# DRL-Navigation/DDRL4NAV

Hardware: NVIDIA B200
Metric: PPO learner samples/s & batched policy actions/s at 1/2/4/8 B200 (higher is better)
Workload: dtype f32 (three tcgen05 kind::f16 products of scaled fp16 hi/lo splits, fp32 accumulate)

## Files before the change

### ddrl4nav_b200/_lib.py

```python
import ctypes as C
import os

_HERE = os.path.dirname(os.path.abspath(__file__))
LIB_PATH = os.environ.get("DDRL_LIB_PATH") or os.path.join(_HERE, "libddrl_b200.so")


class DDRLError(RuntimeError):
    pass


class NetDesc(C.Structure):
    _fields_ = [("arch", C.c_int32), ("in_ch", C.c_int32), ("act_dim", C.c_int32), ("dist", C.c_int32),
                ("shared", C.c_int32), ("feat", C.c_int32), ("gemm_mode", C.c_int32), ("laser_ch", C.c_int32)]


class PPOHparams(C.Structure):
    _fields_ = [("ppo_clip", C.c_float), ("dual_clip", C.c_float), ("v_coef", C.c_float), ("ent_coef", C.c_float),
                ("max_grad_norm", C.c_float), ("clip_grad", C.c_int32), ("smooth_l1", C.c_int32),
                ("lr", C.c_float), ("lr_actor", C.c_float), ("lr_critic", C.c_float),
                ("beta1", C.c_float), ("beta2", C.c_float), ("adam_eps", C.c_float)]


class GatherJob(C.Structure):
    _fields_ = [("src", C.c_void_p), ("dst", C.c_void_p), ("row_bytes", C.c_int64), ("src_stride", C.c_int64),
# ... 44 lines not shown
    "ddrl_net_num_params": (_L, [_P]),
    "ddrl_net_tensor_info": (_I, [_P, _I, C.c_char_p, _I, C.POINTER(_L), C.POINTER(_I), C.POINTER(_L)]),
    "ddrl_net_bind": (_I, [_P, _P, _P, _P, _P]),
    "ddrl_net_params_changed": (_I, [_P]),
    "ddrl_net_set_extra_critics": (_I, [_P, _I, C.POINTER(_P), C.POINTER(_P), C.POINTER(_P), C.POINTER(_P), C.POINTER(_I)]),
    "ddrl_net_num_obs": (_I, [_P]),
    "ddrl_net_obs_elems": (_L, [_P, _I]),
    "ddrl_net_forward": (_I, [_P, C.POINTER(_P), _I, _I, _P, _P, _P, _P, _P, _P]),
    "ddrl_net_encode": (_I, [_P, C.POINTER(_P), _I, _I, _I, _P, _P]),
    "ddrl_net_backward": (_I, [_P, C.POINTER(_P), _I, _I, _I, _P, _P, _P, _P, C.POINTER(PPOHparams), _I, _P]),
    "ddrl_net_backward_segment": (_I, [_P, C.POINTER(_P), _I, _I, _I, _P, _P, _P, _P, C.POINTER(PPOHparams), _I, _I, C.POINTER(_I), _P]),
    "ddrl_net_tensor_segment": (_I, [_P, _I]),
    "ddrl_net_backward_minibatch": (_I, [_P, C.POINTER(_P), _I, _I, _I, _P, _P, _P, _P, C.POINTER(PPOHparams), _P]),
    "ddrl_gather_rows": (_I, [_P, _I, C.POINTER(GatherJob), _I, _P]),
    "ddrl_set_deterministic": (_I, [_I]),
    "ddrl_peer_allreduce_flag_bytes": (_I, []),
    "ddrl_peer_allreduce_f32": (_I, [C.POINTER(_P), _P, C.POINTER(_P), _I, _I, C.c_int64, C.c_int64, C.c_uint32, _P]),
    "ddrl_net_clip_adam": (_I, [_P, _I, C.POINTER(PPOHparams), _P, _P]),
    "ddrl_net_workspace_bytes": (_L, [_P]),
}

_lib = None


def load():
    global _lib
    if _lib is not None:
        return _lib
    if not os.path.exists(LIB_PATH):
        raise DDRLError(
# ... 34 lines not shown
```

### ddrl4nav_b200/csrc/tc3.cu

```cuda
#include <cuda.h>
#include <cuda_fp16.h>

#include <algorithm>
#include <cstdlib>
#include <cstring>
#include <mutex>
#include <vector>

#include "common.cuh"
#include "layer_ops.h"
#include "prep_kernels.cuh"
#include "tc_ptx.cuh"

namespace ddrl {

constexpr int T3_BM = 128;
constexpr int T3_BK = 64;
constexpr int T3_CHUNK = 4;

__device__ unsigned long long g_tc3_wait[96];
#ifdef TC3_TIMING
#define T3_T0 const long long _t0 = clock64()
#define T3_ACC(acc) acc += clock64() - _t0
#define T3_WAIT(bar, par, acc) do { T3_T0; mbar_wait(bar, par); T3_ACC(acc); } while (0)
// ... 31 lines not shown
  int act, atomic, vec_store;
  int tma_store;
  int tma_mask;
  int presplit;
  int b_resident;
  int m_tiles, n_tiles;
  const float* amax_a;
  const float* amax_b;
  float* amax_out;
  unsigned int* bits_out;
  const unsigned int* bits_in;
  float* colsum;
  float* colsum2;
  int colsum_split;
  unsigned int* det_ctr;
  TcTap tap;
};

template <bool SCALED = true>
__device__ __forceinline__ void t3_split2(float x0, float x1, float s, uint32_t& hi, uint32_t& lo) {
  const float y0 = SCALED ? x0 * s : x0, y1 = SCALED ? x1 * s : x1;
  asm("cvt.rn.satfinite.f16x2.f32 %0, %1, %2;" : "=r"(hi) : "f"(y1), "f"(y0));
  const float2 f = __half22float2(*reinterpret_cast<const __half2*>(&hi));
  const float r0 = (y0 - f.x) * T3_LO, r1 = (y1 - f.y) * T3_LO;
  asm("cvt.rn.satfinite.f16x2.f32 %0, %1, %2;" : "=r"(lo) : "f"(r1), "f"(r0));
}

__device__ __forceinline__ void umma_f16_ts(uint32_t tmem_d, uint32_t tmem_a, uint64_t db, uint32_t idesc, uint32_t accumulate) {
  asm volatile(
      "{\n"
      ".reg .pred p;\n"
      "setp.ne.b32 p, %4, 0;\n"
      "tcgen05.mma.cta_group::1.kind::f16 [%0], [%1], %2, %3, p;\n"
      "}" ::"r"(tmem_d), "r"(tmem_a), "l"(db), "r"(idesc), "r"(accumulate) : "memory");
}

__device__ __forceinline__ void umma_f16_ss(uint32_t tmem_d, uint64_t da, uint64_t db, uint32_t idesc, uint32_t accumulate) {
  asm volatile(
      "{\n"
      ".reg .pred p;\n"
      "setp.ne.b32 p, %4, 0;\n"
      "tcgen05.mma.cta_group::1.kind::f16 [%0], %1, %2, %3, p;\n"
      "}" ::"r"(tmem_d), "l"(da), "l"(db), "r"(idesc), "r"(accumulate) : "memory");
}

template <int BN>
struct T3Cfg {
  static constexpr int A_SUB = T3_BM * 128;
  static constexpr int A_BYTES = 2 * A_SUB;
  static constexpr int B_BYTES = BN * 128;
  static constexpr int STAGE_BYTES = A_BYTES + 2 * B_BYTES;
  static constexpr int STAGES = BN <= 32 ? 5 : (BN <= 64 ? 4 : 3);
  static constexpr bool FOLD = BN <= 64;
  static constexpr int SA = BN <= 32 ? 4 : (BN <= 64 ? 3 : 2);
  static constexpr int NEPI = BN <= 32 ? 4 : 8;
  static constexpr int NSG = BN <= 64 ? 2 : 1;
  static constexpr int EPI0 = 4 + 4 * NSG;
  static constexpr int THREADS = (EPI0 + NEPI) * 32;
  static constexpr int COLS = BN / (NEPI / 4);
  static constexpr int TM_MAIN0 = 0, TM_MAIN1 = FOLD ? 2 * BN : BN, TM_CORR = FOLD ? 4 * BN : 2 * BN, TM_A = FOLD ? 5 * BN : 3 * BN;
  static constexpr int TMEM_COLS = 512;
  static constexpr int NBARS = 2 * STAGES + SA + 7;
  static constexpr int STG_OFF = STAGES * STAGE_BYTES;
  static constexpr int BAR_OFF = STG_OFF + NEPI * 4096;
  static constexpr int BIAS_OFF = BAR_OFF + 256;
  static constexpr int SMEM = 1024 + BIAS_OFF + BN * 4;
  static_assert(NBARS * 8 + 16 <= 256, "barrier block");
  static_assert(SMEM <= 232448, "shared memory budget");
  static_assert(TM_A + SA * 64 <= 512, "TMEM budget");
  static_assert(STAGES > SA, "the stage barrier of K block it - SA releases TMEM slot it % SA");
};

template <int BN>
__global__ void __launch_bounds__(T3Cfg<BN>::THREADS, 1)
tc3_kernel(const __grid_constant__ CUtensorMap tmA, const __grid_constant__ CUtensorMap tmBhi,
           const __grid_constant__ CUtensorMap tmBlo, const __grid_constant__ CUtensorMap tmA2,
           const __grid_constant__ CUtensorMap tmC, const __grid_constant__ CUtensorMap tmC2,
           const __grid_constant__ CUtensorMap tmM, const __grid_constant__ CUtensorMap tmM2, Tc3Args g) {
  using Cfg = T3Cfg<BN>;
  constexpr int S = Cfg::STAGES, SA = Cfg::SA;
  extern __shared__ uint8_t smem_dyn[];
  uint8_t* smem = smem_dyn + ((1024u - (smem_u32(smem_dyn) & 1023u)) & 1023u);
  uint64_t* bars = reinterpret_cast<uint64_t*>(smem + Cfg::BAR_OFF);
  uint64_t* bar_full = bars;
  uint64_t* bar_empty = bars + S;
  uint64_t* bar_aready = bars + 2 * S;
  uint64_t* bar_mfull = bars + 2 * S + SA;
  uint64_t* bar_mfree = bar_mfull + 2;
  uint64_t* bar_cfull = bar_mfull + 4;
  uint64_t* bar_cfree = bar_mfull + 5;
  uint64_t* bar_mask = bar_mfull + 6;
  uint32_t* tmem_slot = reinterpret_cast<uint32_t*>(bars + Cfg::NBARS);
  const int warp = threadIdx.x >> 5, lane = threadIdx.x & 31;
  const TcTap& tp = g.tap;
  const bool tapA = tp.mode != 0;

  if (warp == 0 && lane == 0) {
    mbar_init(smem_u32(bar_mask), 1);
    for (int s = 0; s < S; ++s) { mbar_init(smem_u32(bar_full + s), 1); mbar_init(smem_u32(bar_empty + s), 2); }
    for (int a = 0; a < SA; ++a) mbar_init(smem_u32(bar_aready + a), 4);
    for (int b = 0; b < 2; ++b) { mbar_init(smem_u32(bar_mfull + b), 1); mbar_init(smem_u32(bar_mfree + b), Cfg::NEPI); }
    mbar_init(smem_u32(bar_cfull), 1);
    mbar_init(smem_u32(bar_cfree), Cfg::NEPI);
    asm volatile("fence.mbarrier_init.release.cluster;" ::: "memory");
  }
  if (warp == 2) {
    asm volatile("tcgen05.alloc.cta_group::1.sync.aligned.shared::cta.b32 [%0], %1;" ::"r"(smem_u32(tmem_slot)),
                 "r"((uint32_t)Cfg::TMEM_COLS) : "memory");
    asm volatile("tcgen05.relinquish_alloc_permit.cta_group::1.sync.aligned;" ::: "memory");
  }
  tc_fence_before();
  __syncthreads();
  tc_fence_after();
  const uint32_t tmem_base = *tmem_slot;

  const int total_tiles = g.m_tiles * g.n_tiles;
  const int tile_step = (int)gridDim.x, tile_first = (int)blockIdx.x;
  const int nkb = g.kb_total;
  const bool ps = g.presplit != 0;
  const bool odd_tail = tapA && !ps && (tp.nslices & 1);

  if (warp == 0) {
    uint32_t it = 0;
    T3_ROLE_BEGIN
    for (int tile = tile_first; tile < total_tiles; tile += tile_step) {
      const int mt = tile / g.n_tiles, nt = tile - mt * g.n_tiles;
      const int m0 = mt * T3_BM, n0 = nt * BN;
      int b0 = 0, y0 = 0;
      const bool ph2 = tapA && mt >= tp.tiles1;
      if (tapA) {
        if (!ph2) { b0 = (mt / tp.tpi) * tp.nb; y0 = (mt % tp.tpi) * tp.ny * tp.sy - tp.py; }
        else { b0 = (mt - tp.tiles1) * tp.nb2; y0 = tp.y2 * tp.sy - tp.py; }
      }
      int cc = 0, kw = 0, kh = 0;
      for (int i = 0; i < nkb; ++i, ++it) {
        const uint32_t s = it % S;
        T3_WAITL(smem_u32(bar_empty + s), ((it / S) & 1) ^ 1, w0);
        const bool load_b = !g.b_resident || it < (uint32_t)S;
        const uint32_t b_tx = load_b ? 2u * Cfg::B_BYTES : 0u;
        if (elect_one()) {
          const uint32_t full = smem_u32(bar_full + s);
          const uint32_t a_dst = smem_u32(smem) + s * Cfg::STAGE_BYTES, bh_dst = a_dst + Cfg::A_BYTES, bl_dst = bh_dst + Cfg::B_BYTES;
          const int k = i * T3_BK;
          if (ps) {
            if (!tapA) {
              mbar_expect_tx(full, Cfg::A_BYTES + b_tx);
              tma_load_2d(&tmA, full, a_dst, k, m0);
// ... 28 lines not shown
        if (tapA) {
#pragma unroll
          for (int j = 0; j < 2; ++j) {
            if (ps && j == 1) break;
            if (++cc == tp.cpb) { cc = 0; if (++kw == tp.KW) { kw = 0; ++kh; } }
          }
        }
      }
    }
    T3_ROLE_END(0, true);
  } else if (warp == 1 || warp == 3) {
    const bool chunk_role = warp == 1;
    const uint32_t idesc = (1u << 4) | ((uint32_t)(BN >> 3) << 17) | ((uint32_t)(T3_BM >> 4) << 24);
    const uint32_t idesc2 = (1u << 4) | ((uint32_t)((2 * BN) >> 3) << 17) | ((uint32_t)(T3_BM >> 4) << 24);
    const uint32_t smem_base = smem_u32(smem);
    const uint32_t t_corr = tmem_base + Cfg::TM_CORR;
    uint32_t it = 0, ch = 0, tl = 0;
    T3_ROLE_BEGIN
    for (int tile = tile_first; tile < total_tiles; tile += tile_step, ++tl) {
      for (int i = 0; i < nkb; ++i, ++it) {
        const uint32_t s = it % S, a = it % SA;
        const uint32_t buf = ch & 1;
        const bool first_in_chunk = (i % T3_CHUNK) == 0;
        const bool last_in_chunk = (i % T3_CHUNK) == T3_CHUNK - 1 || i == nkb - 1;
        const int ksteps = (odd_tail && i == nkb - 1) ? 2 : 4;
        if (chunk_role) { if (first_in_chunk) T3_WAIT(smem_u32(bar_mfree + buf), ((ch >> 1) & 1) ^ 1, w0); }
        else if (i == 0) T3_WAIT(smem_u32(bar_cfree), (tl & 1) ^ 1, w0);
        if (ps) T3_WAIT(smem_u32(bar_full + s), (it / S) & 1, w1);
        else T3_WAIT(smem_u32(bar_aready + a), (it / SA) & 1, w1);
        tc_fence_after();
        T3_SECTION_BEGIN;
        if (elect_one()) {
          const uint32_t b_hi = smem_base + s * Cfg::STAGE_BYTES + Cfg::A_BYTES, b_lo = b_hi + Cfg::B_BYTES;
          const uint32_t a_hi = tmem_base + Cfg::TM_A + a * 64, a_lo = a_hi + 32;
          const uint64_t dbh0 = umma_desc(b_hi, 16, 1024, 2);
          if (ps) {
            const uint32_t sa_hi = smem_base + s * Cfg::STAGE_BYTES;
            const uint64_t dah0 = umma_desc(sa_hi, 16, 1024, 2), dal0 = umma_desc(sa_hi + Cfg::A_SUB, 16, 1024, 2);
            if (chunk_role) {
              const uint32_t t_main = tmem_base + (buf ? Cfg::TM_MAIN1 : Cfg::TM_MAIN0);
#pragma unroll
              for (int k4 = 0; k4 < 4; ++k4)
                umma_f16_ss(t_main, dah0 + k4 * 2, dbh0 + k4 * 2, Cfg::FOLD ? idesc2 : idesc, (!first_in_chunk || k4 != 0) ? 1u : 0u);
              umma_commit(smem_u32(bar_empty + s));
              if (last_in_chunk) umma_commit(smem_u32(bar_mfull + buf));
            } else {
              const uint64_t dbl0 = umma_desc(b_lo, 16, 1024, 2);
#pragma unroll
              for (int k4 = 0; k4 < 4; ++k4) {
                umma_f16_ss(t_corr, dal0 + k4 * 2, dbh0 + k4 * 2, idesc, (i | k4) != 0 ? 1u : 0u);
                if (!Cfg::FOLD) umma_f16_ss(t_corr, dah0 + k4 * 2, dbl0 + k4 * 2, idesc, 1u);
              }
              umma_commit(smem_u32(bar_empty + s));
              if (i == nkb - 1) umma_commit(smem_u32(bar_cfull));
            }
          } else if (chunk_role) {
            const uint32_t t_main = tmem_base + (buf ? Cfg::TM_MAIN1 : Cfg::TM_MAIN0);
#pragma unroll
            for (int k4 = 0; k4 < 4; ++k4) {
              if (k4 >= ksteps) break;
              umma_f16_ts(t_main, a_hi + k4 * 8, dbh0 + k4 * 2, Cfg::FOLD ? idesc2 : idesc, (!first_in_chunk || k4 != 0) ? 1u : 0u);
            }
            umma_commit(smem_u32(bar_empty + s));
            if (last_in_chunk) umma_commit(smem_u32(bar_mfull + buf));
          } else {
            const uint64_t dbl0 = umma_desc(b_lo, 16, 1024, 2);
#pragma unroll
            for (int k4 = 0; k4 < 4; ++k4) {
              if (k4 >= ksteps) break;
              umma_f16_ts(t_corr, a_lo + k4 * 8, dbh0 + k4 * 2, idesc, (i | k4) != 0 ? 1u : 0u);
              if (!Cfg::FOLD) umma_f16_ts(t_corr, a_hi + k4 * 8, dbl0 + k4 * 2, idesc, 1u);
            }
            umma_commit(smem_u32(bar_empty + s));
            if (i == nkb - 1) umma_commit(smem_u32(bar_cfull));
          }
        }
        __syncwarp();
        T3_SECTION_END(w2);
        if (last_in_chunk) ++ch;
      }
    }
    T3_ROLE_END(chunk_role ? 1 : 2, true);
  } else if (warp >= 4 && warp < Cfg::EPI0) {
    const int q = (warp - 4) & 3, grp = (warp - 4) >> 2;
    const uint32_t t_lane = (uint32_t)(q * 32) << 16;
    float sA, sA_inv;
    t3_scale(__ldg(g.amax_a), sA, sA_inv);
    const bool unit_scale = sA == 1.f;
    const int row = q * 32 + lane;
    uint32_t it = 0;
    T3_ROLE_BEGIN
    for (int tile = ps ? total_tiles : tile_first; tile < total_tiles; tile += tile_step) {
      for (int i = 0; i < nkb; ++i, ++it) {
        const int s = it % S, a = it % SA;
// ... 119 lines not shown
  } else if (warp >= Cfg::EPI0) {
    const int e = warp - Cfg::EPI0;
    const int q = e & 3, half = e >> 2;
    const uint32_t t_lane = (uint32_t)(q * 32) << 16;
    const uint32_t col0 = half * Cfg::COLS;
    float sA, sA_inv, sB, sB_inv;
    t3_scale(__ldg(g.amax_a), sA, sA_inv);
    t3_scale(__ldg(g.amax_b), sB, sB_inv);
    float run_max = 0.f;
    uint32_t ch = 0, tl = 0, mround = 0;
    float s_pre = 1.f, s_out = sA_inv * sB_inv;
    if (!(s_out >= 1e-30f && s_out <= 1e30f)) { s_pre = sA_inv; s_out = sB_inv; }
    const int r = q * 32 + lane;
    int ryb1 = 0, ryb2 = 0;
    const bool need_off = !g.tma_store || g.bits_out != nullptr || g.bits_in != nullptr;
    const int rx = (tapA && need_off) ? r % tp.Xn : 0;
    if (tapA) {
      const int t1 = r / tp.Xn;
      ryb1 = (t1 % tp.ny) | ((t1 / tp.ny) << 16);
      if (tp.ny2 > 0) ryb2 = (t1 % tp.ny2) | ((t1 / tp.ny2) << 16);
    }
    float* bias_s = reinterpret_cast<float*>(smem + Cfg::BIAS_OFF);
    const int et = e * 32 + lane;
    T3_ROLE_BEGIN
    for (int tile = tile_first; tile < total_tiles; tile += tile_step, ++tl) {
      const int mt = tile / g.n_tiles, nt = tile - mt * g.n_tiles;
      const int m0 = mt * T3_BM, n0 = nt * BN;
      int cy = 0, cb = 0;
      if (tapA) {
        const bool ph2 = mt >= tp.tiles1;
        cb = ph2 ? (mt - tp.tiles1) * tp.nb2 : (mt / tp.tpi) * tp.nb;
        cy = ph2 ? tp.y2 : (mt % tp.tpi) * tp.ny;
      }
      const bool masked = g.tma_store && g.tma_mask;
      float bias_r = 0.f;
      if (g.tma_store && et < BN && g.bias != nullptr && n0 + et < g.N) bias_r = __ldg(g.bias + n0 + et);
      const bool ph2e = tapA && mt >= tp.tiles1;
      const int ryb = ph2e ? ryb2 : ryb1;
      const bool rvalid = tapA ? (r < (ph2e ? tp.rows2 : tp.rows) && cb + (ryb >> 16) < tp.Bn && cy + (ryb & 0xffff) < tp.Yn)
                               : (m0 + r) < g.M;
      const bool fused = tapA && tp.ncls > 1;
      long long roff = 0;
      int py = 0, px = 0;
      if (need_off) {
        if (tapA) {
          const int yy = ryb & 0xffff, bb = ryb >> 16;
          roff = (long long)(cb + bb) * tp.osb + (long long)(cy + yy) * tp.osy + (long long)rx * tp.osx;
          if (fused) { px = rx * tp.out_s; py = (cy + yy) * tp.out_s; }
        } else {
          roff = (long long)(m0 + r) * g.sCm;
        }
      }
      uint32_t mw[Cfg::COLS / 32];
#pragma unroll
      for (int p = 0; p < Cfg::COLS / 32; ++p) mw[p] = 0u;
// ... 31 lines not shown
            continue;
          }
          tmem_ld32(tmem_base + t_lane + (buf ? Cfg::TM_MAIN1 : Cfg::TM_MAIN0) + col0 + j0, v);
#pragma unroll
          for (int j = 0; j < 32; ++j) acc[j0 + j] += v[j];
          if (Cfg::FOLD) {
            tmem_ld32(tmem_base + t_lane + (buf ? Cfg::TM_MAIN1 : Cfg::TM_MAIN0) + BN + col0 + j0, v);
#pragma unroll
            for (int j = 0; j < 32; ++j) acc[j0 + j] = fmaf(v[j], T3_LO_INV, acc[j0 + j]);
          }
        }
        tc_fence_before();
        __syncwarp();
        if (lane == 0) mbar_arrive(smem_u32(bar_mfree + buf));
      }
      T3_WAITL(smem_u32(bar_cfull), tl & 1, w1);
      tc_fence_after();
#pragma unroll
      for (int j0 = 0; j0 < Cfg::COLS; j0 += 32) {
        float v[32];
        tmem_ld32(tmem_base + t_lane + Cfg::TM_CORR + col0 + j0, v);
#pragma unroll
        for (int j = 0; j < 32; ++j) acc[j0 + j] = fmaf(v[j], T3_LO_INV, acc[j0 + j]);
      }
      tc_fence_before();
      __syncwarp();
      if (lane == 0) mbar_arrive(smem_u32(bar_cfree));
      if (s_pre != 1.f) {
#pragma unroll
        for (int j = 0; j < Cfg::COLS; ++j) acc[j] *= s_pre;
      }
      T3_SECTION_BEGIN;
      const float neg_slope = g.act == 3 ? 0.f : 0.01f;
      if (!g.tma_store) {
#pragma unroll
        for (int j = 0; j < Cfg::COLS; ++j) acc[j] *= s_out;
      }
      if (g.tma_store) {
        float* stg = reinterpret_cast<float*>(smem + Cfg::STG_OFF) + e * 1024;
        const bool relu = g.act == 1;
        const float slope = g.act == 2 ? 0.01f : 1.f;
        const bool has_bias = g.bias != nullptr;
// ... 219 lines not shown
#pragma unroll
      for (int o = 16; o > 0; o >>= 1) run_max = fmaxf(run_max, __shfl_xor_sync(0xffffffffu, run_max, o));
      if (lane == 0 && run_max > 0.f) atomicMax(reinterpret_cast<unsigned int*>(g.amax_out), __float_as_uint(run_max));
    }
  }
  tc_fence_before();
  __syncthreads();
  if (warp == 2) {
    asm volatile("tcgen05.dealloc.cta_group::1.sync.aligned.b32 %0, %1;" ::"r"(tmem_base), "r"((uint32_t)Cfg::TMEM_COLS)
                 : "memory");
  }
}

struct Tc3Maps { CUtensorMap a, bhi, blo, a2, c, c2, m, m2; };

template <int BN>
static int launch3(const Tc3Maps& m, const Tc3Args& g, dim3 grid, cudaStream_t s) {
  using Cfg = T3Cfg<BN>;
  static bool attr_done_dev[64] = {};
  bool& attr_done = attr_done_dev[current_device_index()];
  if (!attr_done) {
    DDRL_CUDA(cudaFuncSetAttribute(tc3_kernel<BN>, cudaFuncAttributeMaxDynamicSharedMemorySize, Cfg::SMEM));
    attr_done = true;
  }
  static const bool no_bres = [] { const char* e = getenv("DDRL_TC3_NO_BRES"); return e && e[0] == '1'; }();
  Tc3Args ga = g;
  ga.b_resident = (!no_bres && g.n_tiles == 1 && g.kb_total >= 1 && Cfg::STAGES % g.kb_total == 0) ? 1 : 0;
  tc3_kernel<BN><<<grid, Cfg::THREADS, Cfg::SMEM, s>>>(m.a, m.bhi, m.blo, m.a2, m.c, m.c2, m.m, m.m2, ga);
  prof_work(2.0 * g.M * (double)g.N * g.K * (g.tap.work_scale > 0.f ? g.tap.work_scale : 1.f));
  if (g_prof_on && g_prof_shapes) {
    char nm[96];
    snprintf(nm, sizeof(nm), "%s3[fwd,M=%d,N=%d,K=%d,g=%d]", g.tap.mode ? "conv_tc" : "gemm_tc", g.M, g.N, g.K,
             (int)(grid.x * grid.y * grid.z));
    DDRL_LAUNCHED(prof_intern(nm));
    return DDRL_OK;
  }
  DDRL_LAUNCHED("tc3_kernel");
  return DDRL_OK;
}

static int launch3_bn(int bn, const Tc3Maps& m, const Tc3Args& g, dim3 grid, cudaStream_t s) {
  switch (bn) {
    case 128: return launch3<128>(m, g, grid, s);
    case 64: return launch3<64>(m, g, grid, s);
    default: return launch3<32>(m, g, grid, s);
  }
}
static const bool g_t3_tma_store = [] { const char* e = getenv("DDRL_TC3_TMA_STORE"); return !(e && e[0] == '0'); }();
static const bool g_t3_tma_dgrad = [] { const char* e = getenv("DDRL_TC3_TMA_DGRAD"); return !(e && e[0] == '0'); }();

static inline int pick_bn3(int N) { return N > 64 ? 128 : (N > 32 ? 64 : 32); }
static inline bool al16(const void* p) { return (reinterpret_cast<uintptr_t>(p) & 15) == 0; }
// ... 3 lines not shown
  const unsigned long long strides[1] = {(unsigned long long)ldb16 * 2};
  const unsigned box[2] = {64u, (unsigned)bn}, estr[2] = {1u, 1u};
  return tc_encode_tiled(m, true, 2, base, dims, strides, box, estr, true);
}

static int make_map_nhwc16(CUtensorMap* m, const void* plane, const ConvOp& o, int nx, int ny, int nb) {
  const unsigned long long dims[4] = {(unsigned long long)o.Ctot, (unsigned long long)o.Win, (unsigned long long)o.Hin, (unsigned long long)o.Bn};
  const unsigned long long strides[3] = {(unsigned long long)o.Ctot * 2, (unsigned long long)o.Win * o.Ctot * 2,
                                         (unsigned long long)o.Hin * o.Win * o.Ctot * 2};
  const unsigned box[4] = {64u, (unsigned)((nx - 1) * o.sx + 1), (unsigned)((ny - 1) * o.sy + 1), (unsigned)nb};
  const unsigned estr[4] = {1u, (unsigned)o.sx, (unsigned)o.sy, 1u};
  return tc_encode_tiled(m, true, 4, plane, dims, strides, box, estr, true);
}
static inline bool presplit_ok(const ConvOp& o, const void* hi, const void* lo) {
  return hi && lo && al16(hi) && al16(lo) && o.Cin % 64 == 0 && o.Ctot % 8 == 0 && o.c_off % 8 == 0;
}

__global__ void __launch_bounds__(256) presplit_kernel(const float* __restrict__ x, long long n8, const float* __restrict__ amax,
                                                       uint4* __restrict__ hi, uint4* __restrict__ lo) {
  float sA, sA_inv;
  t3_scale(__ldg(amax), sA, sA_inv);
  const float4* x4 = reinterpret_cast<const float4*>(x);
  for (long long i = (long long)blockIdx.x * blockDim.x + threadIdx.x; i < n8; i += (long long)gridDim.x * blockDim.x) {
    const float4 a = __ldg(x4 + 2 * i), b = __ldg(x4 + 2 * i + 1);
    uint4 h, l;
    t3_split2(a.x, a.y, sA, h.x, l.x); t3_split2(a.z, a.w, sA, h.y, l.y);
    t3_split2(b.x, b.y, sA, h.z, l.z); t3_split2(b.z, b.w, sA, h.w, l.w);
    hi[i] = h; lo[i] = l;
  }
}
// ... 100 lines not shown
  const int bn = pick_bn3(N);
  Tc3Args g;
  memset(&g, 0, sizeof(g));
  tc_tap_common(g.tap, o, T3_BM, true);
  g.tap.osb = osb; g.tap.osy = osy; g.tap.osx = osx;
  if (cls && cls->ncls > 1) {
    if (cls->ncls > 4 || N != cls->ncls * cls->cls_cols || cls->cls_cols % 4 != 0) return DDRL_E_ARG;
    g.tap.ncls = cls->ncls; g.tap.cls_cols = cls->cls_cols; g.tap.out_s = cls->out_s; g.tap.out_H = cls->out_H;
    g.tap.out_W = cls->out_W; g.tap.work_scale = cls->work_scale;
    for (int q = 0; q < cls->ncls; ++q) {
      g.tap.cls_iy[q] = cls->cls_iy[q]; g.tap.cls_ix[q] = cls->cls_ix[q]; g.tap.cls_off[q] = cls->cls_off[q];
      if (cls->cls_off[q] % 4 != 0) return DDRL_E_ARG;
    }
  }
  const int K = o.KH * o.KW * o.Cin;
  Tc3Maps mp;
  const bool ph2 = g.tap.ny2 > 0;
  if (ps) {
    g.presplit = 1;
    g.tap.cpb = o.Cin / 64; g.tap.nslices = o.KH * o.KW * g.tap.cpb;
    r = make_map_nhwc16(&mp.a, a_hi16, o, o.Xn, g.tap.ny, g.tap.nb);
    if (r == DDRL_OK && ph2) r = make_map_nhwc16(&mp.a2, a_hi16, o, o.Xn, g.tap.ny2, g.tap.nb2);
  } else {
    r = tc_make_map_nhwc(&mp.a, o, o.Xn, g.tap.ny, g.tap.nb, false);
    if (r == DDRL_OK && ph2) r = tc_make_map_nhwc(&mp.a2, o, o.Xn, g.tap.ny2, g.tap.nb2, false);
  }
  if (r == DDRL_OK) r = make_map_b16(&mp.bhi, Whi, K, N, ldw16, bn);
  if (r == DDRL_OK) r = make_map_b16(&mp.blo, Wlo, K, N, ldw16, bn);
  if (r != DDRL_OK) return r;
  if (!ph2) mp.a2 = mp.a;
  g.C = out; g.bias = bias; g.mask = mask; g.act = act;
  g.M = o.Bn * o.Yn * o.Xn; g.N = N; g.K = K; g.sCm = 0; g.sCn = 1;
  g.kb_total = ps ? g.tap.nslices : (g.tap.nslices + 1) / 2; g.kb_per_split = g.kb_total;
  g.m_tiles = ceil_div(o.Bn, g.tap.nb) * g.tap.tpi + (ph2 ? ceil_div(o.Bn, g.tap.nb2) : 0);
  g.n_tiles = ceil_div(N, bn);
  g.amax_a = amax_a; g.amax_b = amax_b; g.amax_out = amax_out;
  g.vec_store = (osb % 4 == 0 && osy % 4 == 0 && osx % 4 == 0 && al16(out) && (!mask || al16(mask))) ? 1 : 0;
// ... 2 lines not shown
  const bool classes_ok = classes && g_t3_tma_dgrad && g.tap.cls_cols % 32 == 0 && g.tap.out_W > 1 && g.tap.ncls == g.tap.out_s * g.tap.out_s &&
                          ct > 0 && osx == ct * g.tap.out_s && osy == (long long)g.tap.out_s * g.tap.out_W * ct &&
                          osb == (long long)g.tap.out_H * g.tap.out_W * ct;
  const bool tma_ok = g.vec_store && g_t3_tma_store && (act < 3 || g_t3_tma_dgrad) && (!classes || classes_ok);
  const unsigned int* mbits = (tma_ok && act >= 3 && osb % 32 == 0 && osy % 32 == 0 && osx % 32 == 0 && (!classes || g.tap.cls_cols % 32 == 0))
                                  ? signbits_for_mask(mask) : nullptr;
  if (mbits && classes)
    for (int q = 0; q < g.tap.ncls; ++q) if (g.tap.cls_off[q] % 32 != 0) mbits = nullptr;
  if (tma_ok) {
    const int es = classes ? g.tap.out_s : 1;
    const unsigned long long dims[4] = {(unsigned long long)(classes ? g.tap.cls_cols : N), (unsigned long long)(classes ? g.tap.out_W : o.Xn),
                                        (unsigned long long)(classes ? g.tap.out_H : o.Yn), (unsigned long long)o.Bn};
    const unsigned long long strides[3] = {(unsigned long long)(osx / es) * 4, (unsigned long long)(osy / es) * 4, (unsigned long long)osb * 4};
    const unsigned estr[4] = {1u, (unsigned)es, (unsigned)es, 1u};
    auto boxdim = [&](int n) { return (unsigned)((n - 1) * es + 1); };
    const unsigned box1[4] = {32u, boxdim(o.Xn), boxdim(g.tap.ny), (unsigned)g.tap.nb};
    const unsigned box2[4] = {32u, boxdim(o.Xn), boxdim(g.tap.ny2 > 0 ? g.tap.ny2 : 1), (unsigned)(g.tap.nb2 > 0 ? g.tap.nb2 : 1)};
    int rs = tc_encode_tiled(&mp.c, false, 4, out, dims, strides, box1, estr, true);
    if (rs == DDRL_OK && ph2) rs = tc_encode_tiled(&mp.c2, false, 4, out, dims, strides, box2, estr, true);
    if (rs == DDRL_OK && act >= 3 && !mbits) {
      rs = tc_encode_tiled(&mp.m, false, 4, mask, dims, strides, box1, estr, true);
      if (rs == DDRL_OK && ph2) rs = tc_encode_tiled(&mp.m2, false, 4, mask, dims, strides, box2, estr, true);
    }
    if (rs == DDRL_OK) { g.tma_store = 1; g.tma_mask = (act >= 3 && !mbits) ? 1 : 0; g.bits_in = mbits; }
  }
  g.bits_out = signbits_for_output(out, g.tma_store && !classes && (act == 1 || act == 2) && N % 32 == 0 && osx == N &&
                                            osy == (long long)o.Xn * N && osb == (long long)o.Yn * o.Xn * N);
  if (!g.tma_store) mp.c = mp.a;
  if (!g.tma_store || !ph2) mp.c2 = mp.c;
  if (!g.tma_mask) mp.m = mp.c;
  if (!g.tma_mask || !ph2) mp.m2 = mp.m;
  if (ps) {
    r = make_map_nhwc16(&mp.m, a_lo16, o, o.Xn, g.tap.ny, g.tap.nb);
    if (r == DDRL_OK && ph2) r = make_map_nhwc16(&mp.m2, a_lo16, o, o.Xn, g.tap.ny2, g.tap.nb2);
    if (r != DDRL_OK) return r;
    if (!ph2) mp.m2 = mp.m;
  }
  dim3 grid(std::min(g.m_tiles * g.n_tiles, kNumSMs), 1, 1);
  return launch3_bn(bn, mp, g, grid, s);
}

template <int BN>
struct T3WCfg {
  static_assert(BN == 64 || BN == 128, "weight-gradient tiles are 64 or 128 columns");
  static constexpr int R_SUB = T3_BK * 128;
  static constexpr int A_SUB = R_SUB;
  static constexpr int A_BYTES = 4 * A_SUB;
  static constexpr int BRAW_BYTES = (BN / 32) * R_SUB;
  static constexpr int STAGE_BYTES = A_BYTES + BRAW_BYTES;
  static constexpr int B16_TILE = T3_BK * 128;
  static constexpr int B16_BYTES = 2 * (BN / 64) * B16_TILE;
  static constexpr bool FOLD = BN <= 64;
  static constexpr int SA = BN <= 64 ? 3 : 2;
// ... 609 lines not shown
                                          reinterpret_cast<__half*>(hiT), reinterpret_cast<__half*>(loT), ldT16);
  DDRL_LAUNCHED("split_f16_kernel");
  return DDRL_OK;
}

}

extern "C" int ddrl_tc3_timing_read(unsigned long long* out64, int reset) {
  if (out64) DDRL_CUDA(cudaMemcpyFromSymbol(out64, ddrl::g_tc3_wait, sizeof(unsigned long long) * 96));
  if (reset) {
    unsigned long long z[64] = {0};
    DDRL_CUDA(cudaMemcpyToSymbol(ddrl::g_tc3_wait, z, sizeof(z)));
  }
  return DDRL_OK;
}
```

### ddrl4nav_b200/kernels.py

```python
import ctypes as C
from typing import Optional, Sequence

import torch

from . import _lib
from ._lib import DDRLError, PPOHparams, check, current_stream, ptr, require_cuda


def make_hparams(ppo_clip=0.2, dual_clip=3.0, v_coef=1.0, ent_coef=0.05, max_grad_norm=0.5, clip_grad=True,
                 smooth_l1=False, lr=2e-4, lr_actor=5e-5, lr_critic=1e-3, beta1=0.9, beta2=0.999,
                 adam_eps=1e-8) -> PPOHparams:
    return PPOHparams(ppo_clip, dual_clip, v_coef, ent_coef, max_grad_norm, int(bool(clip_grad)), int(bool(smooth_l1)),
                      lr, lr_actor, lr_critic, beta1, beta2, adam_eps)


def _f32c(t: torch.Tensor) -> torch.Tensor:
    require_cuda(t)
    if t.dtype != torch.float32 or not t.is_contiguous():
        t = t.to(torch.float32).contiguous()
    return t


def set_deterministic(on: bool = True) -> bool:
    return bool(_lib.load().ddrl_set_deterministic(1 if on else 0))


def gae(values: torch.Tensor, rewards: torch.Tensor, dones: torch.Tensor, gamma: Sequence[float], lam: float,
        algo: int = 0):
    lib = _lib.load()
    values = _f32c(values)
    rewards = _f32c(rewards)
    require_cuda(dones)
    if dones.dtype != torch.uint8 or not dones.is_contiguous():
        dones = dones.to(torch.uint8).contiguous()
    Tp1, V, N = values.shape
    T = Tp1 - 1
    assert rewards.shape[0] >= T and dones.shape[0] >= T and tuple(rewards.shape[1:]) == (V, N)
    ret = torch.empty((T, V, N), dtype=torch.float32, device=values.device)
    adv = torch.empty((T, N), dtype=torch.float32, device=values.device)
# ... 199 lines not shown
```

### include/ddrl_b200.h

```cpp
#ifndef DDRL_B200_H
#define DDRL_B200_H

#include <stdint.h>

#ifdef __cplusplus
extern "C" {
#endif

#define DDRL_OK 0
#define DDRL_E_ARG (-1)
#define DDRL_E_CUDA (-2)
#define DDRL_E_STATE (-3)
#define DDRL_E_UNSUPPORTED (-4)
#define DDRL_E_NOMEM (-5)

enum ddrl_arch {
  DDRL_ARCH_ATARI = 0,
  DDRL_ARCH_NAV = 1,
  DDRL_ARCH_NAVPED = 2,
  DDRL_ARCH_NAV1D = 3,
  DDRL_ARCH_MLP = 4
};
enum ddrl_dist { DDRL_DIST_CATEGORICAL = 0, DDRL_DIST_GAUSSIAN = 1 };
enum ddrl_gemm_mode {
// ... 24 lines not shown
  float max_grad_norm;
  int32_t clip_grad;
  int32_t smooth_l1;
  float lr;
  float lr_actor;
  float lr_critic;
  float beta1, beta2, adam_eps;
} ddrl_ppo_hparams;

int ddrl_version(void);
const char* ddrl_error_string(int code);
const char* ddrl_last_cuda_error(void);
int64_t ddrl_launch_count(void);
void ddrl_launch_count_reset(void);
int ddrl_set_deterministic(int on);
int ddrl_prof_start(void* stream);
int ddrl_prof_stop(char* out, int cap);

int ddrl_gae_f32(const float* values, const float* rewards, const uint8_t* dones,
                 const float* gamma_host, float lambda, int T, int V, int N,
                 float* ret, float* adv, int algo, void* stream);

int ddrl_gae_tempo(const float* values, const float* rewards, const uint8_t* dones, const int* durations,
                   const double* table_host, int table_len, double lambda, int T, int V, int N,
                   void* ret, void* adv, int out_f64, void* stream);

int ddrl_easybytes_decode(const uint8_t* payload, const void* segs, int nseg, unsigned int max_count, float* dst,
                          void* stream);

int64_t ddrl_easybytes_reply_bytes(int nb, int act_cols, int V);
// ... 84 lines not shown
```

Before: 1.662 million.

## Add halo-tile conv mode loading each input tile once for all filter taps

Adds a HALO variant of the tc3 conv kernel for stride-1, 64-channel, 64-output convs with small filters. It loads a padded input tile once per output tile and forms each tap by shifting the shared-memory descriptor, and keeps the weights resident in shared memory across tiles. This replaces the per-tap TMA loads of A and per-stage B loads. The cost is wasted output rows in the padded pitch, which are masked in the epilogue, plus a double-buffered correction TMEM region with extra barriers. It is enabled by default and can be turned off with an env var or ddrl_set_halo.

Result: faster. 1.689 million (median of 6 runs) (+1.6%).

```diff
diff --git a/ddrl4nav_b200/_lib.py b/ddrl4nav_b200/_lib.py
--- a/ddrl4nav_b200/_lib.py
+++ b/ddrl4nav_b200/_lib.py
@@ -82,6 +82,7 @@
     "ddrl_net_backward_minibatch": (_I, [_P, C.POINTER(_P), _I, _I, _I, _P, _P, _P, _P, C.POINTER(PPOHparams), _P]),
     "ddrl_gather_rows": (_I, [_P, _I, C.POINTER(GatherJob), _I, _P]),
     "ddrl_set_deterministic": (_I, [_I]),
+    "ddrl_set_halo": (_I, [_I]),
     "ddrl_peer_allreduce_flag_bytes": (_I, []),
     "ddrl_peer_allreduce_f32": (_I, [C.POINTER(_P), _P, C.POINTER(_P), _I, _I, C.c_int64, C.c_int64, C.c_uint32, _P]),
     "ddrl_net_clip_adam": (_I, [_P, _I, C.POINTER(PPOHparams), _P, _P]),
diff --git a/ddrl4nav_b200/csrc/tc3.cu b/ddrl4nav_b200/csrc/tc3.cu
--- a/ddrl4nav_b200/csrc/tc3.cu
+++ b/ddrl4nav_b200/csrc/tc3.cu
@@ -69,6 +69,7 @@
   float* colsum2;
   int colsum_split;
   unsigned int* det_ctr;
+  int hp, hb, hb2;
   TcTap tap;
 };
 
@@ -99,40 +100,46 @@
       "}" ::"r"(tmem_d), "l"(da), "l"(db), "r"(idesc), "r"(accumulate) : "memory");
 }
 
-template <int BN>
+template <int BN, bool HALO = false>
 struct T3Cfg {
-  static constexpr int A_SUB = T3_BM * 128;
+  static constexpr int HROWS = 160;
+  static constexpr int HPLANE = HROWS * 128;
+  static constexpr int KBR = 4;
+  static constexpr int A_SUB = HALO ? HPLANE : T3_BM * 128;
   static constexpr int A_BYTES = 2 * A_SUB;
   static constexpr int B_BYTES = BN * 128;
-  static constexpr int STAGE_BYTES = A_BYTES + 2 * B_BYTES;
-  static constexpr int STAGES = BN <= 32 ? 5 : (BN <= 64 ? 4 : 3);
+  static constexpr int STAGE_BYTES = HALO ? A_BYTES : A_BYTES + 2 * B_BYTES;
+  static constexpr int STAGES = HALO ? 3 : (BN <= 32 ? 5 : (BN <= 64 ? 4 : 3));
   static constexpr bool FOLD = BN <= 64;
   static constexpr int SA = BN <= 32 ? 4 : (BN <= 64 ? 3 : 2);
   static constexpr int NEPI = BN <= 32 ? 4 : 8;
   static constexpr int NSG = BN <= 64 ? 2 : 1;
-  static constexpr int EPI0 = 4 + 4 * NSG;
+  static constexpr int EPI0 = 4 + (HALO ? 0 : 4 * NSG);
   static constexpr int THREADS = (EPI0 + NEPI) * 32;
   static constexpr int COLS = BN / (NEPI / 4);
   static constexpr int TM_MAIN0 = 0, TM_MAIN1 = FOLD ? 2 * BN : BN, TM_CORR = FOLD ? 4 * BN : 2 * BN, TM_A = FOLD ? 5 * BN : 3 * BN;
   static constexpr int TMEM_COLS = 512;
-  static constexpr int NBARS = 2 * STAGES + SA + 7;
-  static constexpr int STG_OFF = STAGES * STAGE_BYTES;
+  static constexpr int TM_CORR1 = HALO ? TM_A : TM_CORR;
+  static constexpr int NBARS = 2 * STAGES + SA + 7 + (HALO ? 2 : 0);
+  static constexpr int B_OFF = STAGES * STAGE_BYTES;
+  static constexpr int STG_OFF = B_OFF + (HALO ? KBR * 2 * B_BYTES : 0);
   static constexpr int BAR_OFF = STG_OFF + NEPI * 4096;
   static constexpr int BIAS_OFF = BAR_OFF + 256;
   static constexpr int SMEM = 1024 + BIAS_OFF + BN * 4;
   static_assert(NBARS * 8 + 16 <= 256, "barrier block");
   static_assert(SMEM <= 232448, "shared memory budget");
   static_assert(TM_A + SA * 64 <= 512, "TMEM budget");
-  static_assert(STAGES > SA, "the stage barrier of K block it - SA releases TMEM slot it % SA");
+  static_assert(TM_CORR1 + BN <= 512, "TMEM budget (halo correction buffer)");
+  static_assert(HALO || STAGES > SA, "the stage barrier of K block it - SA releases TMEM slot it % SA");
 };
 
-template <int BN>
-__global__ void __launch_bounds__(T3Cfg<BN>::THREADS, 1)
+template <int BN, bool HALO>
+__global__ void __launch_bounds__(T3Cfg<BN, HALO>::THREADS, 1)
 tc3_kernel(const __grid_constant__ CUtensorMap tmA, const __grid_constant__ CUtensorMap tmBhi,
            const __grid_constant__ CUtensorMap tmBlo, const __grid_constant__ CUtensorMap tmA2,
            const __grid_constant__ CUtensorMap tmC, const __grid_constant__ CUtensorMap tmC2,
            const __grid_constant__ CUtensorMap tmM, const __grid_constant__ CUtensorMap tmM2, Tc3Args g) {
-  using Cfg = T3Cfg<BN>;
+  using Cfg = T3Cfg<BN, HALO>;
   constexpr int S = Cfg::STAGES, SA = Cfg::SA;
   extern __shared__ uint8_t smem_dyn[];
   uint8_t* smem = smem_dyn + ((1024u - (smem_u32(smem_dyn) & 1023u)) & 1023u);
@@ -144,6 +151,12 @@
   uint64_t* bar_mfree = bar_mfull + 2;
   uint64_t* bar_cfull = bar_mfull + 4;
   uint64_t* bar_cfree = bar_mfull + 5;
+  auto corr_bars = [&](uint32_t tl, uint64_t*& full, uint64_t*& free_, uint32_t& phase) {
+    const bool odd = HALO && (tl & 1);
+    full = odd ? bar_mfull + 7 : bar_cfull;
+    free_ = odd ? bar_mfull + 8 : bar_cfree;
+    phase = HALO ? (tl >> 1) & 1 : tl & 1;
+  };
   uint64_t* bar_mask = bar_mfull + 6;
   uint32_t* tmem_slot = reinterpret_cast<uint32_t*>(bars + Cfg::NBARS);
   const int warp = threadIdx.x >> 5, lane = threadIdx.x & 31;
@@ -157,6 +170,7 @@
     for (int b = 0; b < 2; ++b) { mbar_init(smem_u32(bar_mfull + b), 1); mbar_init(smem_u32(bar_mfree + b), Cfg::NEPI); }
     mbar_init(smem_u32(bar_cfull), 1);
     mbar_init(smem_u32(bar_cfree), Cfg::NEPI);
+    if (HALO) { mbar_init(smem_u32(bar_mfull + 7), 1); mbar_init(smem_u32(bar_mfull + 8), Cfg::NEPI); }
     asm volatile("fence.mbarrier_init.release.cluster;" ::: "memory");
   }
   if (warp == 2) {
@@ -176,9 +190,9 @@
   const bool odd_tail = tapA && !ps && (tp.nslices & 1);
 
   if (warp == 0) {
-    uint32_t it = 0;
+    uint32_t it = 0, tl = 0;
     T3_ROLE_BEGIN
-    for (int tile = tile_first; tile < total_tiles; tile += tile_step) {
+    for (int tile = tile_first; tile < total_tiles; tile += tile_step, ++tl) {
       const int mt = tile / g.n_tiles, nt = tile - mt * g.n_tiles;
       const int m0 = mt * T3_BM, n0 = nt * BN;
       int b0 = 0, y0 = 0;
@@ -186,6 +200,27 @@
       if (tapA) {
         if (!ph2) { b0 = (mt / tp.tpi) * tp.nb; y0 = (mt % tp.tpi) * tp.ny * tp.sy - tp.py; }
         else { b0 = (mt - tp.tiles1) * tp.nb2; y0 = tp.y2 * tp.sy - tp.py; }
+      }
+      if constexpr (HALO) {
+        const uint32_t s = tl % S;
+        T3_WAITL(smem_u32(bar_empty + s), ((tl / S) & 1) ^ 1, w0);
+        if (elect_one()) {
+          const uint32_t full = smem_u32(bar_full + s);
+          const uint32_t a_dst = smem_u32(smem) + s * Cfg::STAGE_BYTES;
+          const uint32_t box = (uint32_t)(ph2 ? tp.nb2 * g.hb2 : tp.nb * g.hb) * (uint32_t)g.hp * 128u;
+          mbar_expect_tx(full, 2u * box + (tl == 0 ? (uint32_t)nkb * 2u * Cfg::B_BYTES : 0u));
+          tma_load_4d(ph2 ? &tmA2 : &tmA, full, a_dst, tp.c_off, -tp.px, y0, b0);
+          tma_load_4d(ph2 ? &tmM2 : &tmM, full, a_dst + Cfg::A_SUB, tp.c_off, -tp.px, y0, b0);
+          if (tl == 0) {
+            for (int i = 0; i < nkb; ++i) {
+              const uint32_t bh_dst = smem_u32(smem) + Cfg::B_OFF + i * 2 * Cfg::B_BYTES;
+              tma_load_2d(&tmBhi, full, bh_dst, i * T3_BK, n0);
+              tma_load_2d(&tmBlo, full, bh_dst + Cfg::B_BYTES, i * T3_BK, n0);
+            }
+          }
+        }
+        __syncwarp();
+        continue;
       }
       int cc = 0, kw = 0, kh = 0;
       for (int i = 0; i < nkb; ++i, ++it) {
@@ -244,35 +279,42 @@
     const uint32_t idesc = (1u << 4) | ((uint32_t)(BN >> 3) << 17) | ((uint32_t)(T3_BM >> 4) << 24);
     const uint32_t idesc2 = (1u << 4) | ((uint32_t)((2 * BN) >> 3) << 17) | ((uint32_t)(T3_BM >> 4) << 24);
     const uint32_t smem_base = smem_u32(smem);
-    const uint32_t t_corr = tmem_base + Cfg::TM_CORR;
     uint32_t it = 0, ch = 0, tl = 0;
     T3_ROLE_BEGIN
     for (int tile = tile_first; tile < total_tiles; tile += tile_step, ++tl) {
+      int kh = 0, kw = 0;
+      uint64_t *c_full, *c_free;
+      uint32_t c_ph;
+      corr_bars(tl, c_full, c_free, c_ph);
+      const uint32_t t_corr = tmem_base + ((HALO && (tl & 1)) ? Cfg::TM_CORR1 : Cfg::TM_CORR);
       for (int i = 0; i < nkb; ++i, ++it) {
-        const uint32_t s = it % S, a = it % SA;
+        const uint32_t s = HALO ? tl % S : it % S, a = it % SA;
         const uint32_t buf = ch & 1;
         const bool first_in_chunk = (i % T3_CHUNK) == 0;
         const bool last_in_chunk = (i % T3_CHUNK) == T3_CHUNK - 1 || i == nkb - 1;
+        const bool release = !HALO || i == nkb - 1;
         const int ksteps = (odd_tail && i == nkb - 1) ? 2 : 4;
         if (chunk_role) { if (first_in_chunk) T3_WAIT(smem_u32(bar_mfree + buf), ((ch >> 1) & 1) ^ 1, w0); }
-        else if (i == 0) T3_WAIT(smem_u32(bar_cfree), (tl & 1) ^ 1, w0);
-        if (ps) T3_WAIT(smem_u32(bar_full + s), (it / S) & 1, w1);
+        else if (i == 0) T3_WAIT(smem_u32(c_free), c_ph ^ 1, w0);
+        if (HALO) { if (i == 0) T3_WAIT(smem_u32(bar_full + s), (tl / S) & 1, w1); }
+        else if (ps) T3_WAIT(smem_u32(bar_full + s), (it / S) & 1, w1);
         else T3_WAIT(smem_u32(bar_aready + a), (it / SA) & 1, w1);
         tc_fence_after();
         T3_SECTION_BEGIN;
         if (elect_one()) {
-          const uint32_t b_hi = smem_base + s * Cfg::STAGE_BYTES + Cfg::A_BYTES, b_lo = b_hi + Cfg::B_BYTES;
+          const uint32_t b_hi = HALO ? smem_base + Cfg::B_OFF + i * 2 * Cfg::B_BYTES : smem_base + s * Cfg::STAGE_BYTES + Cfg::A_BYTES;
+          const uint32_t b_lo = b_hi + Cfg::B_BYTES;
           const uint32_t a_hi = tmem_base + Cfg::TM_A + a * 64, a_lo = a_hi + 32;
           const uint64_t dbh0 = umma_desc(b_hi, 16, 1024, 2);
           if (ps) {
-            const uint32_t sa_hi = smem_base + s * Cfg::STAGE_BYTES;
+            const uint32_t sa_hi = smem_base + s * Cfg::STAGE_BYTES + (HALO ? (uint32_t)(kh * g.hp + kw) * 128u : 0u);
             const uint64_t dah0 = umma_desc(sa_hi, 16, 1024, 2), dal0 = umma_desc(sa_hi + Cfg::A_SUB, 16, 1024, 2);
             if (chunk_role) {
               const uint32_t t_main = tmem_base + (buf ? Cfg::TM_MAIN1 : Cfg::TM_MAIN0);
 #pragma unroll
               for (int k4 = 0; k4 < 4; ++k4)
                 umma_f16_ss(t_main, dah0 + k4 * 2, dbh0 + k4 * 2, Cfg::FOLD ? idesc2 : idesc, (!first_in_chunk || k4 != 0) ? 1u : 0u);
-              umma_commit(smem_u32(bar_empty + s));
+              if (release) umma_commit(smem_u32(bar_empty + s));
               if (last_in_chunk) umma_commit(smem_u32(bar_mfull + buf));
             } else {
               const uint64_t dbl0 = umma_desc(b_lo, 16, 1024, 2);
@@ -281,8 +323,8 @@
                 umma_f16_ss(t_corr, dal0 + k4 * 2, dbh0 + k4 * 2, idesc, (i | k4) != 0 ? 1u : 0u);
                 if (!Cfg::FOLD) umma_f16_ss(t_corr, dah0 + k4 * 2, dbl0 + k4 * 2, idesc, 1u);
               }
-              umma_commit(smem_u32(bar_empty + s));
-              if (i == nkb - 1) umma_commit(smem_u32(bar_cfull));
+              if (release) umma_commit(smem_u32(bar_empty + s));
+              if (i == nkb - 1) umma_commit(smem_u32(c_full));
             }
           } else if (chunk_role) {
             const uint32_t t_main = tmem_base + (buf ? Cfg::TM_MAIN1 : Cfg::TM_MAIN0);
@@ -302,12 +344,13 @@
               if (!Cfg::FOLD) umma_f16_ts(t_corr, a_hi + k4 * 8, dbl0 + k4 * 2, idesc, 1u);
             }
             umma_commit(smem_u32(bar_empty + s));
-            if (i == nkb - 1) umma_commit(smem_u32(bar_cfull));
+            if (i == nkb - 1) umma_commit(smem_u32(c_full));
           }
         }
         __syncwarp();
         T3_SECTION_END(w2);
         if (last_in_chunk) ++ch;
+        if (HALO && ++kw == tp.KW) { kw = 0; ++kh; }
       }
     }
     T3_ROLE_END(chunk_role ? 1 : 2, true);
@@ -457,11 +500,13 @@
     const int r = q * 32 + lane;
     int ryb1 = 0, ryb2 = 0;
     const bool need_off = !g.tma_store || g.bits_out != nullptr || g.bits_in != nullptr;
-    const int rx = (tapA && need_off) ? r % tp.Xn : 0;
+    const int pitch = HALO ? g.hp : tp.Xn;
+    const int rx = (tapA && (HALO || need_off)) ? r % pitch : 0;
     if (tapA) {
-      const int t1 = r / tp.Xn;
-      ryb1 = (t1 % tp.ny) | ((t1 / tp.ny) << 16);
-      if (tp.ny2 > 0) ryb2 = (t1 % tp.ny2) | ((t1 / tp.ny2) << 16);
+      const int t1 = r / pitch;
+      const int per1 = HALO ? g.hb : tp.ny, per2 = HALO ? g.hb2 : tp.ny2;
+      ryb1 = (t1 % per1) | ((t1 / per1) << 16);
+      if (tp.ny2 > 0) ryb2 = (t1 % per2) | ((t1 / per2) << 16);
     }
     float* bias_s = reinterpret_cast<float*>(smem + Cfg::BIAS_OFF);
     const int et = e * 32 + lane;
@@ -480,8 +525,10 @@
       if (g.tma_store && et < BN && g.bias != nullptr && n0 + et < g.N) bias_r = __ldg(g.bias + n0 + et);
       const bool ph2e = tapA && mt >= tp.tiles1;
       const int ryb = ph2e ? ryb2 : ryb1;
-      const bool rvalid = tapA ? (r < (ph2e ? tp.rows2 : tp.rows) && cb + (ryb >> 16) < tp.Bn && cy + (ryb & 0xffff) < tp.Yn)
-                               : (m0 + r) < g.M;
+      const bool rvalid = !tapA ? (m0 + r) < g.M
+                        : HALO ? (rx < tp.Xn && (ryb & 0xffff) < (ph2e ? tp.ny2 : tp.ny) && (ryb >> 16) < (ph2e ? tp.nb2 : tp.nb) &&
+                                  cb + (ryb >> 16) < tp.Bn && cy + (ryb & 0xffff) < tp.Yn)
+                               : (r < (ph2e ? tp.rows2 : tp.rows) && cb + (ryb >> 16) < tp.Bn && cy + (ryb & 0xffff) < tp.Yn);
       const bool fused = tapA && tp.ncls > 1;
       long long roff = 0;
       int py = 0, px = 0;
@@ -543,18 +590,21 @@
         __syncwarp();
         if (lane == 0) mbar_arrive(smem_u32(bar_mfree + buf));
       }
-      T3_WAITL(smem_u32(bar_cfull), tl & 1, w1);
+      uint64_t *c_full, *c_free;
+      uint32_t c_ph;
+      corr_bars(tl, c_full, c_free, c_ph);
+      T3_WAITL(smem_u32(c_full), c_ph, w1);
       tc_fence_after();
 #pragma unroll
       for (int j0 = 0; j0 < Cfg::COLS; j0 += 32) {
         float v[32];
-        tmem_ld32(tmem_base + t_lane + Cfg::TM_CORR + col0 + j0, v);
+        tmem_ld32(tmem_base + t_lane + ((HALO && (tl & 1)) ? Cfg::TM_CORR1 : Cfg::TM_CORR) + col0 + j0, v);
 #pragma unroll
         for (int j = 0; j < 32; ++j) acc[j0 + j] = fmaf(v[j], T3_LO_INV, acc[j0 + j]);
       }
       tc_fence_before();
       __syncwarp();
-      if (lane == 0) mbar_arrive(smem_u32(bar_cfree));
+      if (lane == 0) mbar_arrive(smem_u32(c_free));
       if (s_pre != 1.f) {
 #pragma unroll
         for (int j = 0; j < Cfg::COLS; ++j) acc[j] *= s_pre;
@@ -804,28 +854,29 @@
 
 struct Tc3Maps { CUtensorMap a, bhi, blo, a2, c, c2, m, m2; };
 
-template <int BN>
+template <int BN, bool HALO = false>
 static int launch3(const Tc3Maps& m, const Tc3Args& g, dim3 grid, cudaStream_t s) {
-  using Cfg = T3Cfg<BN>;
+  using Cfg = T3Cfg<BN, HALO>;
+  static_assert(!HALO || BN == 64, "halo mode is built for N = 64 tiles");
   static bool attr_done_dev[64] = {};
   bool& attr_done = attr_done_dev[current_device_index()];
   if (!attr_done) {
-    DDRL_CUDA(cudaFuncSetAttribute(tc3_kernel<BN>, cudaFuncAttributeMaxDynamicSharedMemorySize, Cfg::SMEM));
+    DDRL_CUDA(cudaFuncSetAttribute(tc3_kernel<BN, HALO>, cudaFuncAttributeMaxDynamicSharedMemorySize, Cfg::SMEM));
     attr_done = true;
   }
   static const bool no_bres = [] { const char* e = getenv("DDRL_TC3_NO_BRES"); return e && e[0] == '1'; }();
   Tc3Args ga = g;
-  ga.b_resident = (!no_bres && g.n_tiles == 1 && g.kb_total >= 1 && Cfg::STAGES % g.kb_total == 0) ? 1 : 0;
-  tc3_kernel<BN><<<grid, Cfg::THREADS, Cfg::SMEM, s>>>(m.a, m.bhi, m.blo, m.a2, m.c, m.c2, m.m, m.m2, ga);
+  ga.b_resident = (!HALO && !no_bres && g.n_tiles == 1 && g.kb_total >= 1 && Cfg::STAGES % g.kb_total == 0) ? 1 : 0;
+  tc3_kernel<BN, HALO><<<grid, Cfg::THREADS, Cfg::SMEM, s>>>(m.a, m.bhi, m.blo, m.a2, m.c, m.c2, m.m, m.m2, ga);
   prof_work(2.0 * g.M * (double)g.N * g.K * (g.tap.work_scale > 0.f ? g.tap.work_scale : 1.f));
   if (g_prof_on && g_prof_shapes) {
     char nm[96];
-    snprintf(nm, sizeof(nm), "%s3[fwd,M=%d,N=%d,K=%d,g=%d]", g.tap.mode ? "conv_tc" : "gemm_tc", g.M, g.N, g.K,
-             (int)(grid.x * grid.y * grid.z));
+    snprintf(nm, sizeof(nm), "%s3[fwd%s,M=%d,N=%d,K=%d,g=%d]", g.tap.mode ? "conv_tc" : "gemm_tc", HALO ? ",halo" : "", g.M, g.N,
+             g.K, (int)(grid.x * grid.y * grid.z));
     DDRL_LAUNCHED(prof_intern(nm));
     return DDRL_OK;
   }
-  DDRL_LAUNCHED("tc3_kernel");
+  DDRL_LAUNCHED(HALO ? "tc3_kernel<64,halo>" : "tc3_kernel");
   return DDRL_OK;
 }
 
@@ -859,6 +910,49 @@
 }
 static inline bool presplit_ok(const ConvOp& o, const void* hi, const void* lo) {
   return hi && lo && al16(hi) && al16(lo) && o.Cin % 64 == 0 && o.Ctot % 8 == 0 && o.c_off % 8 == 0;
+}
+
+static int g_halo_set = -1;
+static bool halo_on() {
+  if (g_halo_set >= 0) return g_halo_set != 0;
+  const char* e = getenv("DDRL_NO_HALO");
+  return !(e && e[0] == '1');
+}
+
+static bool halo_plan(const ConvOp& o, Tc3Args& g) {
+  using Cfg = T3Cfg<64, true>;
+  const int hp = o.Win + 2 * o.px;
+  if (o.sx != 1 || o.sy != 1 || o.Xn != hp - o.KW + 1 || o.Yn != o.Hin + 2 * o.py - o.KH + 1 || hp > 256) return false;
+  if (T3_BM + (o.KH - 1) * hp + o.KW - 1 > Cfg::HROWS) return false;
+  auto max_images = [&](int ny) {
+    const int hb = ny + o.KH - 1;
+    int n = 0;
+    while (n < std::min(o.Bn, 256) && n * hb * hp + (ny - 1) * hp + o.Xn <= T3_BM && (n + 1) * hb * hp <= T3_BM) ++n;
+    return n;
+  };
+  double best = 1e30;
+  TcTap& t = g.tap;
+  for (int ny = o.Yn; ny >= 1; --ny) {
+    const int hb = ny + o.KH - 1;
+    if (hb > 256) continue;
+    const int k = o.Yn / ny, rem = o.Yn - k * ny;
+    const int nb = ny == o.Yn ? max_images(ny) : ((ny - 1) * hp + o.Xn <= T3_BM && hb * hp <= Cfg::HROWS && ny * hp <= T3_BM ? 1 : 0);
+    if (nb < 1) continue;
+    const int nb2 = rem > 0 ? max_images(rem) : 0;
+    if (rem > 0 && nb2 < 1) continue;
+    const double c = (double)k / nb + (rem > 0 ? 1.0 / nb2 : 0.0);
+    if (c < best) {
+      best = c;
+      t.ny = ny; t.nb = nb; t.tpi = k; g.hb = hb;
+      t.y2 = rem > 0 ? k * ny : 0; t.ny2 = rem; t.nb2 = nb2; g.hb2 = rem > 0 ? rem + o.KH - 1 : 0;
+    }
+  }
+  if (best >= 1e30) return false;
+  g.hp = hp;
+  t.tiles1 = t.ny2 > 0 ? ceil_div(o.Bn, t.nb) * t.tpi : 0x7fffffff;
+  t.rows = std::min(T3_BM, t.nb * g.hb * hp);
+  t.rows2 = t.ny2 > 0 ? std::min(T3_BM, t.nb2 * g.hb2 * hp) : 0;
+  return true;
 }
 
 __global__ void __launch_bounds__(256) presplit_kernel(const float* __restrict__ x, long long n8, const float* __restrict__ amax,
@@ -989,13 +1083,16 @@
     }
   }
   const int K = o.KH * o.KW * o.Cin;
+  const bool halo = ps && halo_on() && o.Cin == 64 && bn == 64 && o.KH * o.KW <= T3Cfg<64, true>::KBR && g.tap.ncls <= 1 &&
+                    osb % 4 == 0 && osy % 4 == 0 && osx % 4 == 0 && al16(out) && g_t3_tma_store && halo_plan(o, g);
   Tc3Maps mp;
   const bool ph2 = g.tap.ny2 > 0;
+  const int bx = halo ? g.hp : o.Xn, by1 = halo ? g.hb : g.tap.ny, by2 = halo ? g.hb2 : g.tap.ny2;
   if (ps) {
     g.presplit = 1;
     g.tap.cpb = o.Cin / 64; g.tap.nslices = o.KH * o.KW * g.tap.cpb;
-    r = make_map_nhwc16(&mp.a, a_hi16, o, o.Xn, g.tap.ny, g.tap.nb);
-    if (r == DDRL_OK && ph2) r = make_map_nhwc16(&mp.a2, a_hi16, o, o.Xn, g.tap.ny2, g.tap.nb2);
+    r = make_map_nhwc16(&mp.a, a_hi16, o, bx, by1, g.tap.nb);
+    if (r == DDRL_OK && ph2) r = make_map_nhwc16(&mp.a2, a_hi16, o, bx, by2, g.tap.nb2);
   } else {
     r = tc_make_map_nhwc(&mp.a, o, o.Xn, g.tap.ny, g.tap.nb, false);
     if (r == DDRL_OK && ph2) r = tc_make_map_nhwc(&mp.a2, o, o.Xn, g.tap.ny2, g.tap.nb2, false);
@@ -1028,8 +1125,13 @@
     const unsigned long long strides[3] = {(unsigned long long)(osx / es) * 4, (unsigned long long)(osy / es) * 4, (unsigned long long)osb * 4};
     const unsigned estr[4] = {1u, (unsigned)es, (unsigned)es, 1u};
     auto boxdim = [&](int n) { return (unsigned)((n - 1) * es + 1); };
-    const unsigned box1[4] = {32u, boxdim(o.Xn), boxdim(g.tap.ny), (unsigned)g.tap.nb};
-    const unsigned box2[4] = {32u, boxdim(o.Xn), boxdim(g.tap.ny2 > 0 ? g.tap.ny2 : 1), (unsigned)(g.tap.nb2 > 0 ? g.tap.nb2 : 1)};
+    unsigned box1[4] = {32u, boxdim(o.Xn), boxdim(g.tap.ny), (unsigned)g.tap.nb};
+    unsigned box2[4] = {32u, boxdim(o.Xn), boxdim(g.tap.ny2 > 0 ? g.tap.ny2 : 1), (unsigned)(g.tap.nb2 > 0 ? g.tap.nb2 : 1)};
+    if (halo) {
+      box1[1] = box2[1] = (unsigned)g.hp;
+      if (g.tap.nb > 1) box1[2] = (unsigned)g.hb;
+      if (ph2) box2[2] = (unsigned)g.hb2;
+    }
     int rs = tc_encode_tiled(&mp.c, false, 4, out, dims, strides, box1, estr, true);
     if (rs == DDRL_OK && ph2) rs = tc_encode_tiled(&mp.c2, false, 4, out, dims, strides, box2, estr, true);
     if (rs == DDRL_OK && act >= 3 && !mbits) {
@@ -1038,6 +1140,7 @@
     }
     if (rs == DDRL_OK) { g.tma_store = 1; g.tma_mask = (act >= 3 && !mbits) ? 1 : 0; g.bits_in = mbits; }
   }
+  if (halo && !g.tma_store) return DDRL_E_UNSUPPORTED;
   g.bits_out = signbits_for_output(out, g.tma_store && !classes && (act == 1 || act == 2) && N % 32 == 0 && osx == N &&
                                             osy == (long long)o.Xn * N && osb == (long long)o.Yn * o.Xn * N);
   if (!g.tma_store) mp.c = mp.a;
@@ -1045,12 +1148,13 @@
   if (!g.tma_mask) mp.m = mp.c;
   if (!g.tma_mask || !ph2) mp.m2 = mp.m;
   if (ps) {
-    r = make_map_nhwc16(&mp.m, a_lo16, o, o.Xn, g.tap.ny, g.tap.nb);
-    if (r == DDRL_OK && ph2) r = make_map_nhwc16(&mp.m2, a_lo16, o, o.Xn, g.tap.ny2, g.tap.nb2);
+    r = make_map_nhwc16(&mp.m, a_lo16, o, bx, by1, g.tap.nb);
+    if (r == DDRL_OK && ph2) r = make_map_nhwc16(&mp.m2, a_lo16, o, bx, by2, g.tap.nb2);
     if (r != DDRL_OK) return r;
     if (!ph2) mp.m2 = mp.m;
   }
   dim3 grid(std::min(g.m_tiles * g.n_tiles, kNumSMs), 1, 1);
+  if (halo) return launch3<64, true>(mp, g, grid, s);
   return launch3_bn(bn, mp, g, grid, s);
 }
 
@@ -1690,3 +1794,9 @@
   }
   return DDRL_OK;
 }
+
+extern "C" int ddrl_set_halo(int on) {
+  const int was = ddrl::halo_on() ? 1 : 0;
+  ddrl::g_halo_set = on < 0 ? -1 : (on != 0 ? 1 : 0);
+  return was;
+}
diff --git a/ddrl4nav_b200/kernels.py b/ddrl4nav_b200/kernels.py
--- a/ddrl4nav_b200/kernels.py
+++ b/ddrl4nav_b200/kernels.py
@@ -23,6 +23,10 @@
 
 def set_deterministic(on: bool = True) -> bool:
     return bool(_lib.load().ddrl_set_deterministic(1 if on else 0))
+
+
+def set_halo(on: bool = True) -> bool:
+    return bool(_lib.load().ddrl_set_halo(1 if on else 0))
 
 
 def gae(values: torch.Tensor, rewards: torch.Tensor, dones: torch.Tensor, gamma: Sequence[float], lam: float,
diff --git a/include/ddrl_b200.h b/include/ddrl_b200.h
--- a/include/ddrl_b200.h
+++ b/include/ddrl_b200.h
@@ -62,6 +62,7 @@
 int64_t ddrl_launch_count(void);
 void ddrl_launch_count_reset(void);
 int ddrl_set_deterministic(int on);
+int ddrl_set_halo(int on);
 int ddrl_prof_start(void* stream);
 int ddrl_prof_stop(char* out, int cap);
 
```
